# yeeus/GCI

Measured on AMD Instinct MI355X. Metric: aligned Gbases/s through filter+depth pipeline (CHM13, 40x HiFi), higher is better.
Workload: dtype int32

## Files before the change

### gci_amd/csrc/gci_wave.hpp

```cpp
#pragma once
#include <hip/hip_runtime.h>
#include <stdint.h>

template <int CTRL, int ROW_MASK>
__device__ __forceinline__ int32_t dpp_add(int32_t v)
{
    return v + __builtin_amdgcn_update_dpp(0, v, CTRL, ROW_MASK, 0xF, true);
}

__device__ __forceinline__ int32_t wave_inclusive_i32(int32_t v)
{
    v = dpp_add<0x111, 0xF>(v);
    v = dpp_add<0x112, 0xF>(v);
    v = dpp_add<0x114, 0xF>(v);
    v = dpp_add<0x118, 0xF>(v);
    v = dpp_add<0x142, 0xA>(v);
    v = dpp_add<0x143, 0xC>(v);
    return v;
}

template <typename T>
__device__ __forceinline__ T wave_inclusive(T v, int lane)
{
    if constexpr (sizeof(T) == 4) {
        return (T)wave_inclusive_i32((int32_t)v);
    } else {
#pragma unroll
        for (int d = 1; d < 64; d <<= 1) { T n = __shfl_up(v, d, 64); if (lane >= d) v += n; }
        return v;
    }
}

template <typename T>
__device__ __forceinline__ T wave_sum(T v)
{
    if constexpr (sizeof(T) == 4) {
        return (T)__builtin_amdgcn_readlane(wave_inclusive_i32((int32_t)v), 63);
    } else {
#pragma unroll
        for (int m = 32; m >= 1; m >>= 1) v += __shfl_xor(v, m, 64);
        return v;
    }
}

template <typename T, int NWAVES>
__device__ __forceinline__ T block_exclusive(T v, T* wtot, T& total)
{
    const int t = threadIdx.x, lane = t & 63, wave = t >> 6;
    const T inc = wave_inclusive<T>(v, lane);
    if (lane == 63) wtot[wave] = inc;
    __syncthreads();
    T pre = inc - v, all = 0;
#pragma unroll
    for (int w = 0; w < NWAVES; w++) { if (w < wave) pre += wtot[w]; all += wtot[w]; }
    total = all;
    return pre;
}
```

### gci_amd/csrc/k_filter.hip

```cpp
#include "gci_ctx.hpp"
#include <stdlib.h>

#ifndef G
#define G 4
#endif
#define NSLOT 10
#define LONG_OPS 512u
#ifndef HEAD
#define HEAD 112
#endif
#ifndef AUXB
#define AUXB 112
#endif
#define HEADP (HEAD + 16)
#define AUXP (AUXB + 16)
#define ROW (HEADP + AUXP)
#ifndef KB
#define KB 128
#endif
#ifndef NUP
#define NUP 8
#endif
#ifndef K1_WAVES
#define K1_WAVES 6
#endif
#if G == 4
#define GRP_STEPS(op) do { op(1); op(2); } while (0)
#else
#define GRP_STEPS(op) do { op(1); } while (0)
#endif

#define PIECES 8
#define CHUNK_DW (64 * PIECES * 4)

struct LongItem {
    uint64_t ops_off;
    uint32_t n_ops;
    uint32_t rec;
    int64_t nm;
    int32_t pos, contig, l_seq, n_cigar_field;
    uint32_t mapq;
    uint32_t n_chunks;
    uint32_t chunk_base;
    uint32_t pad;
};

struct ChunkSums { unsigned long long v[5]; };

struct LongQueue {
    uint32_t* next_counters;
    unsigned long long* status_in;
    unsigned long long* next_status;
    uint32_t* n_slow;
    unsigned long long* n_long;
    uint32_t* slow_list;
    LongItem* items;
    unsigned long long* chunks;
    ChunkSums* sums;
    uint32_t cap_items, cap_chunks;
    uint32_t has_seq;
};

__device__ __forceinline__ void report(unsigned long long* status, uint32_t rec, int code)
{
    atomicMin(status, ((unsigned long long)rec << 8) | (unsigned long long)(uint8_t)(-code));
}

__device__ __forceinline__ bool has_zero_byte(uint32_t x) { return ((x - 0x01010101u) & ~x & 0x80808080u) != 0; }

__device__ __forceinline__ bool ratio_cmp(int64_t a, int64_t b, double c, bool le)
{
    if (((a < 0 ? -a : a) | b) >> 30 == 0) {
        const float x = (float)(int32_t)a * __builtin_amdgcn_rcpf((float)(int32_t)b);
        const float cf = (float)c, m = 1e-4f * fmaxf(1.0f, fabsf(x));
        if (c == c && fabs(c) < 1e30) {
            if (x < cf - m) return le;
            if (x > cf + m) return !le;
        }
    }
    const double q = (double)a / (double)b;
    return le ? q <= c : q >= c;
}

__device__ __forceinline__ int decide4(gci_rec& r, int64_t S, int64_t den1, int64_t den2, int64_t rlen, bool have_nm,
                                       bool nm_bad_type, int64_t NM, int32_t pos, int32_t contig, int32_t l_seq,
                                       uint32_t n_cigar_field, int mapq, int mq_cutoff, double clip_percent,
                                       double iden_percent)
{
    if (!have_nm) return GCI_E_NO_NM;
    if (nm_bad_type) return GCI_E_BAD_NM_TYPE;
    if (den1 == 0) return GCI_E_ZERO_DIV;
    if (!ratio_cmp(S, den1, clip_percent, true)) return GCI_OK;
    if (den2 == 0) return GCI_E_ZERO_DIV;
    if (!ratio_cmp(den2 - NM, den2, iden_percent, false)) return GCI_OK;
    if (n_cigar_field == 0) return GCI_E_NO_END;
    r.contig = contig;
    r.start = pos;
    r.end = (int32_t)((int64_t)pos + (rlen > 0 ? rlen : 1));
    r.qlen = l_seq;
    r.flags = GCI_REC_PASS | (mapq >= mq_cutoff ? GCI_REC_HQ : 0);
    return GCI_OK;
}

__device__ __forceinline__ int decide(gci_rec& r, int64_t M, int64_t I, int64_t D, int64_t N, int64_t S, bool have_nm,
                                      bool nm_bad_type, int64_t NM, int32_t pos, int32_t contig, int32_t l_seq,
                                      uint32_t n_cigar_field, int mapq, int mq_cutoff, double clip_percent,
                                      double iden_percent)
{
    return decide4(r, S, M + I + S, M + I + D, M + D + N, have_nm, nm_bad_type, NM, pos, contig, l_seq, n_cigar_field, mapq, mq_cutoff,
                   clip_percent, iden_percent);
}

template <typename P>
__device__ __forceinline__ bool nm_value(P t, int64_t& NM)
{
    uint32_t w = 0;
    switch (t[0]) {
    case 'c': NM = (int8_t)t[1]; return true;
    case 'C': NM = t[1]; return true;
    case 's': w = (uint32_t)t[1] | ((uint32_t)t[2] << 8); NM = (int16_t)w; return true;
    case 'S': w = (uint32_t)t[1] | ((uint32_t)t[2] << 8); NM = w; return true;
    case 'i': w = (uint32_t)t[1] | ((uint32_t)t[2] << 8) | ((uint32_t)t[3] << 16) | ((uint32_t)t[4] << 24); NM = (int32_t)w; return true;
    case 'I': w = (uint32_t)t[1] | ((uint32_t)t[2] << 8) | ((uint32_t)t[3] << 16) | ((uint32_t)t[4] << 24); NM = w; return true;
    default: return false;
    }
}

__device__ __forceinline__ uint4 load16_tail(const uint8_t* __restrict__ bam, uint64_t at, uint64_t n_bytes)
{
    uint32_t w[4] = {0, 0, 0, 0};
#pragma unroll
    for (int i = 0; i < 16; i++) if (at + i < n_bytes) w[i >> 2] |= (uint32_t)bam[at + i] << (8 * (i & 3));
    return make_uint4(w[0], w[1], w[2], w[3]);
}

__device__ __forceinline__ void stage16(uint8_t* dst, const uint8_t* __restrict__ bam, uint64_t at, uint64_t n_bytes)
{
    uint4 v = make_uint4(0, 0, 0, 0);
    if (at + 16 <= n_bytes) v = *reinterpret_cast<const uint4*>(bam + at);
    else if (at < n_bytes) {
        v = load16_tail(bam, at, n_bytes);
    }
    *reinterpret_cast<uint4*>(dst) = v;
}

__device__ __forceinline__ uint32_t lds_u32(const uint8_t* p) { uint32_t v; __builtin_memcpy(&v, p, 4); return v; }

__device__ __forceinline__ void wave_lds_fence()
{
    __builtin_amdgcn_fence(__ATOMIC_RELEASE, "wavefront");
    __builtin_amdgcn_wave_barrier();
    __builtin_amdgcn_fence(__ATOMIC_ACQUIRE, "wavefront");
}

template <int W>
__device__ __forceinline__ bool enqueue_long(const LongQueue& q, LongItem it, int li)
{
    const uint32_t d0 = (uint32_t)(it.ops_off & 15ull) >> 2;
    const uint32_t nch = (uint32_t)(((uint64_t)d0 + it.n_ops + CHUNK_DW - 1) / CHUNK_DW);
    uint32_t slot, base;
    if (W == 64) {
        unsigned long long old = 0;
        if (li == 0) old = atomicAdd(q.n_long, (1ull << 32) | nch);
        slot = (uint32_t)__shfl((int)(old >> 32), 0, 64);
        base = (uint32_t)__shfl((int)(uint32_t)old, 0, 64);
    } else {
        const int lane = threadIdx.x & 63;
        const unsigned long long leaders = __ballot(li == 0);
        uint32_t items_below = 0, chunks_below = 0, chunks_all = 0;
        for (unsigned long long m = leaders; m; m &= m - 1ull) {
            const int l = __builtin_ctzll(m);
            const uint32_t v = (uint32_t)__shfl((int)nch, l, 64);
            if (l < (lane & ~(W - 1))) { items_below++; chunks_below += v; }
            chunks_all += v;
        }
        const int first = __builtin_ctzll(leaders);
        unsigned long long old = 0;
        if (lane == first) old = atomicAdd(q.n_long, ((unsigned long long)__builtin_popcountll(leaders) << 32) | chunks_all);
        slot = (uint32_t)__shfl((int)(old >> 32), first, 64) + items_below;
        base = (uint32_t)__shfl((int)(uint32_t)old, first, 64) + chunks_below;
    }
    const bool ok = slot < q.cap_items && (uint64_t)base + nch <= q.cap_chunks;
    if (li == 0 && slot < q.cap_items) {
        it.n_chunks = ok ? nch : 0u; it.chunk_base = base; it.pad = 0;
        q.items[slot] = it;
    }
    for (uint32_t c = li; c < nch; c += W)
        if ((uint64_t)base + c < q.cap_chunks) q.chunks[base + c] = ok ? ((unsigned long long)slot << 32) | c : ~0ull;
    return ok;
}


__device__ __forceinline__ void cigar_totals_wave(const uint8_t* __restrict__ bam, uint64_t n_bytes, uint64_t p0,
                                                  uint32_t n_ops, int lane, int64_t (&tot)[NSLOT])
{
    long long sum[NSLOT];
#pragma unroll
    for (int k = 0; k < NSLOT; k++) sum[k] = 0;
    const uint32_t sh = (uint32_t)(p0 & 15ull), d = sh >> 2, b = sh & 3u;
    const uint64_t a0 = p0 & ~15ull, lim = n_bytes & ~15ull;
    for (uint32_t c0 = lane; 4ull * c0 < n_ops; c0 += 256) {
        uint4 lo[4], hi[4];
#pragma unroll
        for (int u = 0; u < 4; u++) {
            const uint32_t c = c0 + 64u * u;
            const uint64_t a = a0 + 16ull * c;
            const bool in = 4ull * c < n_ops;
            lo[u] = !in ? make_uint4(0, 0, 0, 0) : a < lim ? *reinterpret_cast<const uint4*>(bam + a) : load16_tail(bam, a, n_bytes);
            hi[u] = !in ? make_uint4(0, 0, 0, 0) : a + 16 < lim ? *reinterpret_cast<const uint4*>(bam + a + 16) : load16_tail(bam, a + 16, n_bytes);
        }
#pragma unroll
        for (int u = 0; u < 4; u++) {
            const uint32_t c = c0 + 64u * u;
            if (4ull * c >= n_ops) continue;
            const uint32_t w[8] = {lo[u].x, lo[u].y, lo[u].z, lo[u].w, hi[u].x, hi[u].y, hi[u].z, hi[u].w};
            const uint32_t m = min(4u, n_ops - 4u * c);
#pragma unroll
            for (int j = 0; j < 4; j++) {
                const uint32_t x0 = d == 0 ? w[j] : d == 1 ? w[j + 1] : d == 2 ? w[j + 2] : w[j + 3];
                const uint32_t x1 = d == 0 ? w[j + 1] : d == 1 ? w[j + 2] : d == 2 ? w[j + 3] : w[j + 4];
                const uint32_t v = __builtin_amdgcn_alignbyte(x1, x0, b);
                const uint32_t op = v & 0xFu;
                const long long len = (uint32_t)j < m ? (long long)(v >> 4) : 0;
#pragma unroll
                for (int q = 0; q < NSLOT - 1; q++) sum[q] += op == (uint32_t)q ? len : 0;
            }
        }
    }
#pragma unroll
    for (int k = 0; k < NSLOT - 1; k++) tot[k] = wave_sum<long long>(sum[k]);
    tot[NSLOT - 1] = 0;
}


__device__ __forceinline__ uint32_t rd16b(const uint8_t* p) { return (uint32_t)p[0] | ((uint32_t)p[1] << 8); }
__device__ __forceinline__ uint32_t rd32b(const uint8_t* p) { return rd16b(p) | (rd16b(p + 2) << 16); }

__device__ __forceinline__ int64_t aux_value_size(const uint8_t* p, const uint8_t* end, uint8_t t)
{
    switch (t) {
    case 'A': case 'c': case 'C': return 1;
    case 's': case 'S': return 2;
    case 'i': case 'I': case 'f': return 4;
    case 'Z': case 'H': {
        const uint8_t* q = p;
        while (q < end && *q) q++;
        return q < end ? (q - p) + 1 : -1;
    }
    case 'B': {
        if (p + 5 > end) return -1;
        const uint8_t sub = p[0];
        const int64_t n = rd32b(p + 1);
        const int64_t es = (sub == 'c' || sub == 'C') ? 1 : (sub == 's' || sub == 'S') ? 2
                         : (sub == 'i' || sub == 'I' || sub == 'f') ? 4 : -1;
        return es < 0 ? -1 : 5 + n * es;
    }
    default: return -1;
    }
}

template <bool QUEUE_ALL = false>
__device__ __forceinline__ void slow_record(
    const uint8_t* __restrict__ bam, uint64_t n_bytes, const uint64_t off,
    const int32_t* __restrict__ ref_sel, uint32_t rec, int lane, const LongQueue& lq, int mq_cutoff, double clip_percent,
    double iden_percent, uint32_t rec_idx_base, gci_rec* __restrict__ out)
{
    const uint8_t* p = bam + off;
    const int32_t block_size = (int32_t)rd32b(p);
    const int32_t ref_id = (int32_t)rd32b(p + 4);
    const int32_t pos = (int32_t)rd32b(p + 8);
    const uint32_t l_read_name = p[12];
    const int mapq = p[13];
    const uint32_t n_cigar = rd16b(p + 16);
    const int32_t l_seq = (int32_t)rd32b(p + 20);
    const int32_t contig = ref_sel[ref_id];
    const uint8_t* name = p + 36;
    const uint8_t* rec_end = p + 4 + block_size;
    const uint8_t* cig = name + l_read_name;
    const uint8_t* aux = cig + 4 * (uint64_t)n_cigar + (lq.has_seq ? (((uint64_t)(uint32_t)l_seq + 1) >> 1) + (uint64_t)(uint32_t)l_seq : 0ull);
    uint32_t nul = l_read_name;
    for (uint32_t i = lane; i < l_read_name; i += 64) if (name[i] == 0) { nul = i; break; }
#pragma unroll
    for (int m = 32; m >= 1; m >>= 1) nul = min(nul, (uint32_t)__shfl_xor((int)nul, m, 64));
    const uint32_t name_len = nul;
    uint64_t acc = 0;
    for (uint32_t k = lane; k * 8 < name_len; k += 64) {
        uint64_t w = 0;
        for (int b = 0; b < 8; b++) if (k * 8 + b < name_len) w |= (uint64_t)name[k * 8 + b] << (8 * b);
        acc += gci_hash_word(w, k);
    }
    acc = (uint64_t)wave_sum<long long>((long long)acc);
    const uint8_t* nm_p = nullptr;
    const uint8_t* cg_p = nullptr;
    for (const uint8_t* q = aux; q + 3 <= rec_end;) {
        const int64_t sz = aux_value_size(q + 3, rec_end, q[2]);
        if (sz < 0 || q + 3 + sz > rec_end) break;
        if (q[0] == 'N' && q[1] == 'M' && !nm_p) nm_p = q + 2;
        if (q[0] == 'C' && q[1] == 'G' && !cg_p) cg_p = q + 2;
        q += 3 + sz;
// ... 247 lines not shown
    GRP_STEPS(STEP_ACC);
#undef STEP_ACC
    r.name_hash = gci_hash_finish(acc, name_len);
    r.name_len = (uint16_t)name_len;

    TR(6);
    if (long_cigar) {
        LongItem it;
        it.ops_off = off + cig_at; it.n_ops = n_cigar; it.rec = rec;
        it.nm = have_nm ? (nm_bad ? INT64_MIN : NM) : INT64_MAX;
        it.pos = pos; it.contig = contig; it.l_seq = l_seq; it.n_cigar_field = (int32_t)n_cigar;
        it.mapq = (uint32_t)mapq;
        if (gl == 0) out[rec] = r;
        if (!enqueue_long<G>(lq, it, gl) && gl == 0) report(lq.status_in, rec, GCI_E_CAPACITY);
        return false;
    }
#define GRP_SUM(x) do { x += (unsigned long long)__shfl_xor((long long)x, 1, G); if (G == 4) x += (unsigned long long)__shfl_xor((long long)x, 2, G); } while (0)
    GRP_SUM(sS); GRP_SUM(sQ); GRP_SUM(sA); GRP_SUM(sR);
#undef GRP_SUM
    if (gl != 0) return false;
    const int st = decide4(r, (int64_t)sS, (int64_t)sQ, (int64_t)sA, (int64_t)sR, have_nm, nm_bad, NM, pos, contig, l_seq,
                           n_cigar, mapq, mq_cutoff, clip_percent, iden_percent);
    if (st != GCI_OK) report(lq.status_in, rec, st);
    out[rec] = r;
    TR(7);
    return false;
    };
    const bool is_slow = live && fast_path();
    for (unsigned long long m = __ballot(is_slow && gl == 0); m; m &= m - 1ull) {
        const uint32_t rs = (uint32_t)__shfl((int)rec, __builtin_ctzll(m), 64);
        slow_record(bam, n_bytes, rec_off[rs], ref_sel, rs, t & 63, lq, mq_cutoff, clip_percent, iden_percent, rec_idx_base, out);
    }
}


__device__ __forceinline__ unsigned long long wave_sum_u40(unsigned long long v)
{
    const uint32_t lo = wave_sum<uint32_t>((uint32_t)v & 0xFFFFu);
    const uint32_t hi = wave_sum<uint32_t>((uint32_t)(v >> 16));
    return (unsigned long long)lo + ((unsigned long long)hi << 16);
}

__global__ __launch_bounds__(BLOCK) void k_cigar_chunks(const uint8_t* __restrict__ bam, uint64_t n_bytes, const LongQueue lq,
                                                        unsigned long long* __restrict__ status)
{
    if (blockIdx.x == 0 && threadIdx.x == 0) *status = *lq.status_in;
    const int lane = threadIdx.x & 63;
    const uint32_t n = (uint32_t)min((unsigned long long)(uint32_t)*lq.n_long, (unsigned long long)lq.cap_chunks);
    const uint32_t waves = gridDim.x * (BLOCK / 64);
    for (uint32_t wi = blockIdx.x * (BLOCK / 64) + (threadIdx.x >> 6); wi < n; wi += waves) {
        const unsigned long long e = lq.chunks[wi];
        if (e == ~0ull) continue;
        const LongItem* it = lq.items + (uint32_t)(e >> 32);
        const uint32_t ci = (uint32_t)e;
        const uint64_t p0 = it->ops_off;
        const uint32_t n_ops = it->n_ops;
        const uint32_t d0 = (uint32_t)(p0 & 15ull) >> 2, b = (uint32_t)p0 & 3u;
        const uint64_t g0 = (uint64_t)ci * CHUNK_DW;
        const uint64_t abase = (p0 & ~15ull) + g0 * 4ull;
        const uint32_t r0 = ci == 0 ? d0 : 0u;
        const uint32_t r1 = (uint32_t)min((uint64_t)CHUNK_DW, (uint64_t)d0 + n_ops - g0);
        uint4 pc[PIECES];
#pragma unroll
        for (int u = 0; u < PIECES; u++) {
            const uint32_t c = lane + 64u * u;
            const uint64_t at = abase + 16ull * c;
            const bool need = 4u * c < r1 + 1u && 4u * c + 4u > r0;
            pc[u] = !need ? make_uint4(0, 0, 0, 0) : at + 16 <= n_bytes ? *reinterpret_cast<const uint4*>(bam + at)
                                                                          : load16_tail(bam, at, n_bytes);
        }
        uint32_t ext = 0;
        if (r1 == CHUNK_DW && b != 0) {
            const uint64_t at = abase + 4ull * CHUNK_DW;
            ext = at + 4 <= n_bytes ? *reinterpret_cast<const uint32_t*>(bam + at) : load16_tail(bam, at, n_bytes).x;
        }
        unsigned long long wide[5] = {0ull, 0ull, 0ull, 0ull, 0ull};
        uint32_t s[5] = {0u, 0u, 0u, 0u, 0u};
#pragma unroll
        for (int u = 0; u < PIECES; u++) {
            uint32_t w4 = (uint32_t)__shfl((int)pc[u].x, (lane + 1) & 63, 64);
            const uint32_t first_next = u + 1 < PIECES ? (uint32_t)__builtin_amdgcn_readfirstlane((int)pc[(u + 1) % PIECES].x) : ext;
            if (lane == 63) w4 = first_next;
            const uint32_t w[5] = {pc[u].x, pc[u].y, pc[u].z, pc[u].w, w4};
            const uint32_t li0 = 4u * (lane + 64u * u);
#pragma unroll
            for (int j = 0; j < 4; j++) {
                const uint32_t v = __builtin_amdgcn_alignbyte(w[j + 1], w[j], b);
                const uint32_t len = (li0 + j - r0) < (r1 - r0) ? v >> 4 : 0u;
                const uint32_t op = v & 0xFu;
                s[0] += len & (0u - ((0x181u >> op) & 1u));
                s[1] += op == 1u ? len : 0u;
                s[2] += op == 2u ? len : 0u;
                s[3] += op == 3u ? len : 0u;
                s[4] += op == 4u ? len : 0u;
            }
            if ((u & 3) == 3) {
#pragma unroll
                for (int k = 0; k < 5; k++) { wide[k] += s[k]; s[k] = 0u; }
            }
        }
        ChunkSums out;
#pragma unroll
        for (int k = 0; k < 5; k++) out.v[k] = wave_sum_u40(wide[k]);
        if (lane == 0) lq.sums[wi] = out;
    }
}

__global__ __launch_bounds__(BLOCK) void k_cigar_finish(const LongQueue lq, int mq_cutoff, double clip_percent,
                                                        double iden_percent, gci_rec* __restrict__ out,
                                                        unsigned long long* __restrict__ status)
{
    const uint32_t n = (uint32_t)min(*lq.n_long >> 32, (unsigned long long)lq.cap_items);
    for (uint32_t i = blockIdx.x * BLOCK + threadIdx.x; i < n; i += gridDim.x * BLOCK) {
        const LongItem x = lq.items[i];
        if (x.n_chunks == 0) continue;
        int64_t t[5] = {0, 0, 0, 0, 0};
        for (uint32_t c = 0; c < x.n_chunks; c++) {
            const ChunkSums cs = lq.sums[x.chunk_base + c];
#pragma unroll
            for (int k = 0; k < 5; k++) t[k] += (int64_t)cs.v[k];
        }
        gci_rec r = out[x.rec];
        const int st = decide(r, t[0], t[1], t[2], t[3], t[4], x.nm != INT64_MAX, x.nm == INT64_MIN, x.nm, x.pos, x.contig,
                              x.l_seq, (uint32_t)x.n_cigar_field, (int)(x.mapq & 0xFFu), mq_cutoff, clip_percent, iden_percent);
        if (st != GCI_OK) report(status, x.rec, st);
        if (r.flags) r.flags |= (uint8_t)(x.mapq >> 8);
        out[x.rec] = r;
    }
}

#define PGK 256
#define PG_KIND_EXT 1u
#define PG_KIND_OVERSIZE 2u
#define PG_KIND_MALFORMED 4u
#define PG_MAGIC 0x31504347u
#define PG_REF_LDS 1024

struct PagesArgs {
    const uint8_t* buf; uint64_t total_bytes; uint32_t page_bytes, n_pages, n_rec;
    const int32_t* ref_sel; int32_t n_ref; int map_qual, mq_cutoff; double clip_percent, iden_percent;
    uint32_t rec_idx_base; gci_rec* out; uint64_t* name_off;
};

#ifndef PG_LPR
#define PG_LPR 4
#endif
#ifndef PG_WAVES
#define PG_WAVES 5
#endif
__global__ __launch_bounds__(PGK) __attribute__((amdgpu_waves_per_eu(PG_WAVES, PG_WAVES))) void k_bam_filter_pages(const PagesArgs A, const LongQueue lq)
{
    extern __shared__ __attribute__((aligned(16))) uint8_t page[];
    __shared__ uint8_t aux_sz[256];
    __shared__ uint8_t aux_kind[256];
    __shared__ uint16_t s_full[GCI_PAGE_MAX_BYTES / 48];
    __shared__ uint32_t s_n_full;
    __shared__ int32_t s_ref_sel[PG_REF_LDS];
    const int t = threadIdx.x;
    const bool ref_in_lds = A.n_ref <= PG_REF_LDS;
    if (ref_in_lds) for (int i = t; i < A.n_ref; i += PGK) s_ref_sel[i] = A.ref_sel[i];
    if (t == 0) s_n_full = 0;
    if (blockIdx.x == 0 && t < 4) lq.next_counters[t] = 0u;
    if (blockIdx.x == 0 && t == 4) *lq.next_status = ~0ull;
    const uint32_t P = A.page_bytes;
    const uint64_t page_at = (uint64_t)blockIdx.x * P;
    {
        const uint4* __restrict__ src = reinterpret_cast<const uint4*>(A.buf + page_at);
        const uint32_t rounds = P / (16u * PGK);
        for (uint32_t r0 = 0; r0 < rounds; r0 += 8) {
            uint4 v[8];
#pragma unroll
            for (int u = 0; u < 8; u++) v[u] = r0 + u < rounds ? src[(r0 + u) * PGK + t] : make_uint4(0, 0, 0, 0);
#pragma unroll
            for (int u = 0; u < 8; u++) if (r0 + u < rounds) reinterpret_cast<uint4*>(page)[(r0 + u) * PGK + t] = v[u];
        }
    }
    for (int i = t; i < 256; i += PGK) {
        const char c = (char)i;
        aux_sz[i] = (c == 'A' || c == 'c' || c == 'C') ? 1 : (c == 's' || c == 'S') ? 2 : (c == 'i' || c == 'I' || c == 'f') ? 4 : 0;
        aux_kind[i] = aux_sz[i] | ((c == 'c' || c == 's' || c == 'i') ? 8 : 0) | ((c == 'c' || c == 'C' || c == 's' || c == 'S' || c == 'i' || c == 'I') ? 16 : 0);
    }
    __syncthreads();
    const uint32_t* ph = reinterpret_cast<const uint32_t*>(page);
    uint32_t n_recs = ph[0];
    const uint32_t first_rec = ph[1];
    if (ph[3] != PG_MAGIC || n_recs > (P - 16u) / 50u || (uint64_t)first_rec + n_recs > A.n_rec) {
        if (t == 0) report(lq.status_in, first_rec < A.n_rec ? first_rec : 0u, GCI_E_MALFORMED);
        n_recs = 0;
    }
    {
        const int tv = PG_LPR == 4 ? t : (int)(((uint32_t)t + 64u * (blockIdx.x & 3u)) & (PGK - 1u));
        const int gl = tv % PG_LPR;
        const uint32_t lgrp = (uint32_t)tv / PG_LPR;
        for (uint32_t j0 = 0; j0 < n_recs; j0 += PGK / PG_LPR) {
            const uint32_t j = j0 + lgrp;
            const uint32_t rec = first_rec + j;
            auto lean_path = [&]() -> int {
                uint32_t base = (uint32_t)reinterpret_cast<const uint16_t*>(page + 16)[j] << 4;
                if (base > P - 48u) return 1;
                const uint8_t* hd = page + base;
                const uint4 c0 = *reinterpret_cast<const uint4*>(hd);
                const uint4 c1 = *reinterpret_cast<const uint4*>(hd + 16);
                const uint32_t size = c0.x, kind = c0.w >> 16, l_read_name = c0.w & 0xFFu, n_cigar = c1.x & 0xFFFFu, flag = c1.x >> 16;
                const int32_t ref_id = (int32_t)c0.y, pos = (int32_t)c0.z, l_seq = (int32_t)c1.y;
                const int mapq = (int)((c0.w >> 8) & 0xFFu);
                const uint32_t aux_len = c1.z;
                const uint32_t cig_at = (36u + l_read_name + 15u) & ~15u;
                const uint32_t aux_at = cig_at + ((4u * n_cigar + 15u) & ~15u);
                if (kind != 0 || l_read_name == 0 || n_cigar == 0 || (uint64_t)aux_at + aux_len > size || base + size > P) return 1;
                gci_rec r;
                r.name_hash = 0; r.contig = -1; r.start = 0; r.end = 0; r.qlen = 0; r.rec_idx = rec + A.rec_idx_base;
                r.mapq = (uint8_t)mapq; r.flags = 0; r.name_len = 0;
                if (gl == 0 && A.name_off) A.name_off[rec] = page_at + base + 36u;
                int32_t contig = -1;
                if (!(ref_id < 0 || ref_id >= A.n_ref || (flag & (0x4u | 0x100u | 0x800u)) || mapq < A.map_qual))
                    contig = ref_in_lds ? s_ref_sel[ref_id] : A.ref_sel[ref_id];
                if (contig < 0) {
                    if (gl == 0) A.out[rec] = r;
                    return 0;
                }
                const uint32_t op0 = lds_u32(hd + cig_at);
                if (pos >= 0 && (op0 & 0xFu) == 4u && (op0 >> 4) == (uint32_t)l_seq) return 1;
                uint32_t sS = 0, sQ = 0, sA = 0, sR = 0, big = 0;
                auto add_op = [&](uint32_t v) {
                    const uint32_t op = v & 0xFu, len = v >> 4;
                    sS = __umul24(len, __builtin_amdgcn_ubfe(0x010u, op, 1)) + sS;
                    sQ = __umul24(len, __builtin_amdgcn_ubfe(0x193u, op, 1)) + sQ;
                    sA = __umul24(len, __builtin_amdgcn_ubfe(0x187u, op, 1)) + sA;
                    sR = __umul24(len, __builtin_amdgcn_ubfe(0x18Du, op, 1)) + sR;
                };
                {
                    const uint8_t* cg = hd + cig_at;
                    for (uint32_t p = gl; 4u * p < n_cigar; p += PG_LPR) {
                        const uint4 v = *reinterpret_cast<const uint4*>(cg + 16u * p);
                        big |= v.x | v.y | v.z | v.w;
                        add_op(v.x); add_op(v.y); add_op(v.z); add_op(v.w);
                    }
                }
                const uint8_t* ax = hd + aux_at;
                uint32_t q = 0, nmk = 0;
                for (;;) {
                    if (q + 3 > aux_len) return 1;
                    const uint32_t w = lds_u32(ax + q);
                    const uint32_t k = aux_kind[(w >> 16) & 0xFFu];
                    if ((k & 7u) == 0 || q + 3 + (k & 7u) > aux_len) return 1;
                    if ((w & 0xFFFFu) == (uint32_t)('N' | ('M' << 8))) { nmk = k; break; }
                    q += 3 + (k & 7u);
                }
                if (!(nmk & 16u)) return 1;
                const uint32_t nv = lds_u32(ax + q + 3), nbits = 8u * (nmk & 7u);
                const int64_t NM = nbits == 32u ? ((nmk & 8u) ? (int64_t)(int32_t)nv : (int64_t)nv)
                                                : ((nmk & 8u) ? (int64_t)__builtin_amdgcn_sbfe((int)nv, 0, nbits) : (int64_t)__builtin_amdgcn_ubfe(nv, 0, nbits));
                const uint8_t* name = hd + 36;
                const uint32_t name_len = l_read_name - 1u;
                bool odd = name[name_len] != 0;
                uint64_t acc = 0;
                for (uint32_t k = gl; k * 8 < name_len; k += PG_LPR) {
                    const uint32_t b0 = k * 8;
                    uint64_t w;
                    __builtin_memcpy(&w, name + b0, 8);
                    const uint32_t keep = name_len - b0;
                    if (keep < 8) w &= (1ull << (8 * keep)) - 1ull;
                    const uint64_t full = keep < 8 ? w | (~0ull << (8 * keep)) : w;
                    odd = odd || (((full - 0x0101010101010101ull) & ~full & 0x8080808080808080ull) != 0);
                    acc += gci_hash_word(w, k);
                }
#pragma unroll
                for (int m = 1; m < PG_LPR; m <<= 1) acc += (uint64_t)__shfl_xor((long long)acc, m, PG_LPR);
                big |= odd ? 0xF0000000u : 0u;
#pragma unroll
                for (int m = 1; m < PG_LPR; m <<= 1) big |= (uint32_t)__shfl_xor((int)big, m, PG_LPR);
                if (big >> 28) return 1;
#define PG_SUM32(x) do { _Pragma("unroll") for (int m = 1; m < PG_LPR; m <<= 1) x += (uint32_t)__shfl_xor((int)x, m, PG_LPR); } while (0)
                PG_SUM32(sS); PG_SUM32(sQ); PG_SUM32(sA); PG_SUM32(sR);
#undef PG_SUM32
                const int64_t num2 = (int64_t)sA - NM;
                if (sQ == 0 || sA == 0 || (sQ >> 30) || (sA >> 30) || num2 > (1 << 30) || num2 < -(1 << 30)) return 1;
                const float x1 = (float)sS * __builtin_amdgcn_rcpf((float)sQ), c1f = (float)A.clip_percent;
                const float x2 = (float)(int32_t)num2 * __builtin_amdgcn_rcpf((float)sA), c2f = (float)A.iden_percent;
                const float m1 = 1e-4f * fmaxf(1.0f, fabsf(x1)), m2 = 1e-4f * fmaxf(1.0f, fabsf(x2));
                if (!(fabs(A.clip_percent) < 1e30) || !(fabs(A.iden_percent) < 1e30)) return 1;
                if (!(x1 < c1f - m1 || x1 > c1f + m1)) return 1;
                r.name_hash = gci_hash_finish(acc, name_len);
                r.name_len = (uint16_t)name_len;
                if (x1 < c1f - m1) {
                    if (!(x2 < c2f - m2 || x2 > c2f + m2)) return 1;
                    if (x2 > c2f + m2) {
                        r.contig = contig; r.start = pos;
                        r.end = (int32_t)((int64_t)pos + (sR > 0 ? (int64_t)sR : 1));
                        r.qlen = l_seq;
                        r.flags = GCI_REC_PASS | (mapq >= A.mq_cutoff ? GCI_REC_HQ : 0) | GCI_REC_NAME16;
                    }
                }
                if (gl == 0) A.out[rec] = r;
                return 0;
            };

            if (j < n_recs && lean_path() != 0 && gl == 0) s_full[atomicAdd(&s_n_full, 1u)] = (uint16_t)j;
        }
    }
    __syncthreads();
    const uint32_t n_full = s_n_full;
    const int gl = t & 3, grp = t >> 2;
    for (uint32_t q0 = 0; q0 < n_full; q0 += PGK / 4) {
        const uint32_t qi = q0 + grp;
        const bool on = qi < n_full;
        const uint32_t j = on ? s_full[qi] : 0u;
        const uint32_t rec = first_rec + j;
        uint64_t slow_off = 0;
        auto fast_path = [&]() -> bool {
            uint32_t base = (uint32_t)reinterpret_cast<const uint16_t*>(page + 16)[j] << 4;
            if (base > P - 48u) base = P - 48u;
            const uint8_t* hd = page + base;
            const uint4 c0 = *reinterpret_cast<const uint4*>(hd);
            const uint4 c1 = *reinterpret_cast<const uint4*>(hd + 16);
            const uint32_t blob_hi = *reinterpret_cast<const uint32_t*>(hd + 32);
            const uint32_t size = c0.x, kind = c0.w >> 16, l_read_name = c0.w & 0xFFu, n_cigar = c1.x & 0xFFFFu, flag = c1.x >> 16;
            const int32_t ref_id = (int32_t)c0.y, pos = (int32_t)c0.z, l_seq = (int32_t)c1.y;
            const int mapq = (int)((c0.w >> 8) & 0xFFu);
            const uint32_t aux_len = c1.z;
            const uint64_t blob_at = (uint64_t)c1.w | ((uint64_t)blob_hi << 32);
            gci_rec r;
            r.name_hash = 0; r.contig = -1; r.start = 0; r.end = 0; r.qlen = 0; r.rec_idx = rec + A.rec_idx_base;
            r.mapq = (uint8_t)mapq; r.flags = 0; r.name_len = 0;
            if (gl == 0 && A.name_off) A.name_off[rec] = (kind == PG_KIND_OVERSIZE ? blob_at : page_at + base) + 36u;
            const bool ext = kind == PG_KIND_EXT;
            const uint32_t cig_at = (36u + l_read_name + 15u) & ~15u;
            const uint32_t aux_at = cig_at + (ext ? 16u : (4u * n_cigar + 15u) & ~15u);
            if ((kind & PG_KIND_MALFORMED) || (kind != PG_KIND_OVERSIZE && ((uint64_t)aux_at + aux_len > size || base + size > P))) {
                if (gl == 0) { report(lq.status_in, rec, GCI_E_MALFORMED); A.out[rec] = r; }
                return false;
            }
            if (ref_id < 0 || ref_id >= A.n_ref || (flag & (0x4u | 0x100u | 0x800u)) || mapq < A.map_qual) {
                if (gl == 0) A.out[rec] = r;
                return false;
            }
            const int32_t contig = ref_in_lds ? s_ref_sel[ref_id] : A.ref_sel[ref_id];
            if (contig < 0) {
                if (gl == 0) A.out[rec] = r;
                return false;
            }
            if (kind == PG_KIND_OVERSIZE) {
                if (blob_at + 36 > A.total_bytes) { if (gl == 0) { report(lq.status_in, rec, GCI_E_MALFORMED); A.out[rec] = r; } return false; }
                slow_off = blob_at;
                return true;
            }
            uint32_t sS = 0, sQ = 0, sA = 0, sR = 0, big = 0;
            auto add_op = [&](uint32_t v) {
                const uint32_t op = v & 0xFu, len = v >> 4;
                sS = __umul24(len, __builtin_amdgcn_ubfe(0x010u, op, 1)) + sS;
                sQ = __umul24(len, __builtin_amdgcn_ubfe(0x193u, op, 1)) + sQ;
                sA = __umul24(len, __builtin_amdgcn_ubfe(0x187u, op, 1)) + sA;
                sR = __umul24(len, __builtin_amdgcn_ubfe(0x18Du, op, 1)) + sR;
            };
            if (!ext) {
                const uint8_t* cg = hd + cig_at;
                for (uint32_t p = gl; 4u * p < n_cigar; p += 4) {
                    const uint4 v = *reinterpret_cast<const uint4*>(cg + 16u * p);
                    big |= v.x | v.y | v.z | v.w;
                    add_op(v.x); add_op(v.y); add_op(v.z); add_op(v.w);
                }
            }
            const uint8_t* ax = hd + aux_at;
            const uint32_t op0 = lds_u32(hd + cig_at);
            const bool want_cg = n_cigar > 0 && pos >= 0 && (op0 & 0xFu) == 4u && (op0 >> 4) == (uint32_t)l_seq;
            bool have_nm = false, nm_bad = false;
            int64_t NM = 0;
            uint32_t cg_q = 0xFFFFFFFFu;
            uint32_t q = 0;
            bool general = want_cg;
            while (!general && q + 3 <= aux_len) {
                const uint32_t w = lds_u32(ax + q);
                const uint32_t sz = aux_sz[(w >> 16) & 0xFFu];
                if (sz == 0) { general = true; break; }
                if (q + 3 + sz > aux_len) break;
                if ((w & 0xFFFFu) == (uint32_t)('N' | ('M' << 8))) { have_nm = true; nm_bad = !nm_value(ax + q + 2, NM); break; }
                q += 3 + sz;
            }
            for (; general && q + 3 <= aux_len;) {
                const uint32_t w = lds_u32(ax + q);
                const uint32_t tag = w & 0xFFFFu;
                const uint8_t ty = (uint8_t)(w >> 16);
                uint32_t sz = aux_sz[ty];
                if (sz == 0) {
                    if (ty == 'Z' || ty == 'H') {
                        uint32_t e = q + 3;
                        while (e < aux_len && ax[e]) e++;
                        if (e >= aux_len) break;
                        sz = e - (q + 3) + 1;
                    } else if (ty == 'B') {
                        if (q + 8 > aux_len) break;
                        const uint8_t sub = ax[q + 3];
                        const uint32_t es = (sub == 'c' || sub == 'C') ? 1u : (sub == 's' || sub == 'S') ? 2u
                                          : (sub == 'i' || sub == 'I' || sub == 'f') ? 4u : 0u;
                        const uint64_t s64 = 5ull + (uint64_t)lds_u32(ax + q + 4) * es;
                        if (es == 0 || s64 > aux_len) break;
                        sz = (uint32_t)s64;
                    } else break;
                }
                if (q + 3 + sz > aux_len) break;
                if (tag == (uint32_t)('N' | ('M' << 8)) && !have_nm) {
                    have_nm = true;
                    nm_bad = !nm_value(ax + q + 2, NM);
                    if (!want_cg || cg_q != 0xFFFFFFFFu) break;
                }
                if (want_cg && tag == (uint32_t)('C' | ('G' << 8)) && cg_q == 0xFFFFFFFFu) {
                    cg_q = q + 2;
                    if (have_nm) break;
                }
                q += 3 + sz;
            }
            bool restored = false;
            if (cg_q != 0xFFFFFFFFu && ax[cg_q] == 'B' && (ax[cg_q + 1] == 'I' || ax[cg_q + 1] == 'i')) {
                const uint32_t cg_len = lds_u32(ax + cg_q + 2);
                if (cg_len >= n_cigar && cg_len < (1u << 29)) {
                    restored = true;
                    sS = sQ = sA = sR = 0; big = 0;
                    for (uint32_t k = gl; k < cg_len; k += 4) { const uint32_t v = lds_u32(ax + cg_q + 6 + 4 * k); big |= v; add_op(v); }
                }
            }
            const uint8_t* name = hd + 36;
            uint32_t nul = l_read_name;
            for (uint32_t i = gl * 4; i < l_read_name; i += 16) {
                if (has_zero_byte(lds_u32(name + i))) {
                    for (uint32_t b = i; b < i + 4 && b < l_read_name; b++) if (name[b] == 0) { nul = min(nul, b); break; }
                    break;
                }
            }
            nul = min(nul, (uint32_t)__shfl_xor((int)nul, 1, 4));
            nul = min(nul, (uint32_t)__shfl_xor((int)nul, 2, 4));
            const uint32_t name_len = nul;
            uint64_t acc = 0;
            for (uint32_t k = gl; k * 8 < name_len; k += 4) {
                const uint32_t b0 = k * 8;
                uint64_t w;
                __builtin_memcpy(&w, name + b0, 8);
                const uint32_t keep = name_len - b0;
                if (keep < 8) w &= (1ull << (8 * keep)) - 1ull;
                acc += gci_hash_word(w, k);
            }
            acc += (uint64_t)__shfl_xor((long long)acc, 1, 4);
            acc += (uint64_t)__shfl_xor((long long)acc, 2, 4);
            r.name_hash = gci_hash_finish(acc, name_len);
            r.name_len = (uint16_t)name_len;
            const uint8_t name16 = name_len + 1u == l_read_name ? GCI_REC_NAME16 : 0;
            big |= (uint32_t)__shfl_xor((int)big, 1, 4);
            big |= (uint32_t)__shfl_xor((int)big, 2, 4);
            const bool wide = (big >> 28) != 0 && !restored;
            if ((ext && !restored) || wide) {
                LongItem it;
                it.ops_off = ext ? blob_at : page_at + base + cig_at; it.n_ops = n_cigar; it.rec = rec;
                it.nm = have_nm ? (nm_bad ? INT64_MIN : NM) : INT64_MAX;
                it.pos = pos; it.contig = contig; it.l_seq = l_seq; it.n_cigar_field = (int32_t)n_cigar;
                it.mapq = (uint32_t)mapq | ((uint32_t)name16 << 8);
                r.flags = 0;
                if (gl == 0) A.out[rec] = r;
                if (it.ops_off + 4ull * n_cigar > A.total_bytes) { if (gl == 0) report(lq.status_in, rec, GCI_E_MALFORMED); return false; }
                if (!enqueue_long<4>(lq, it, gl) && gl == 0) report(lq.status_in, rec, GCI_E_CAPACITY);
                return false;
            }
            unsigned long long tS = sS, tQ = sQ, tA = sA, tR = sR;
            if ((big >> 28) != 0) {
                tS = tQ = tA = tR = 0;
                const uint32_t cg_len = lds_u32(ax + cg_q + 2);
                for (uint32_t k = gl; k < cg_len; k += 4) {
                    const uint32_t v = lds_u32(ax + cg_q + 6 + 4 * k), op = v & 0xFu;
                    const unsigned long long len = v >> 4;
                    tS += len & (0ull - ((0x010u >> op) & 1u)); tQ += len & (0ull - ((0x193u >> op) & 1u));
                    tA += len & (0ull - ((0x187u >> op) & 1u)); tR += len & (0ull - ((0x18Du >> op) & 1u));
                }
            }
#define PG_SUM(x) do { x += (unsigned long long)__shfl_xor((long long)x, 1, 4); x += (unsigned long long)__shfl_xor((long long)x, 2, 4); } while (0)
            PG_SUM(tS); PG_SUM(tQ); PG_SUM(tA); PG_SUM(tR);
#undef PG_SUM
            if (gl != 0) return false;
            const int st = decide4(r, (int64_t)tS, (int64_t)tQ, (int64_t)tA, (int64_t)tR, have_nm, nm_bad, NM, pos, contig, l_seq,
                                   n_cigar, mapq, A.mq_cutoff, A.clip_percent, A.iden_percent);
            if (st != GCI_OK) report(lq.status_in, rec, st);
            if (r.flags) r.flags |= name16;
            A.out[rec] = r;
            return false;
        };
        const bool is_slow = on && fast_path();
        for (unsigned long long m = __ballot(is_slow && gl == 0); m; m &= m - 1ull) {
            const int l = __builtin_ctzll(m);
            const uint32_t rs = (uint32_t)__shfl((int)rec, l, 64);
            const uint64_t so = (uint64_t)__shfl((long long)slow_off, l, 64);
            slow_record<true>(A.buf, A.total_bytes, so, A.ref_sel, rs, t & 63, lq, A.mq_cutoff, A.clip_percent, A.iden_percent, A.rec_idx_base, A.out);
        }
    }
// ... 116 lines not shown
```

Baseline: 24260.

## Restructure lean BAM filter path with batched LDS loads and quad DPP reductions

Rewrites the per-record lean filter path so all LDS loads (contig lookup, first CIGAR op, first CIGAR vector, aux word, NM value, name terminator, first name word) are issued up front and held in registers with clamped addresses. CIGAR and name loops are software-pipelined with prefetch of the next element. Group reductions use quad DPP swizzles instead of shfl_xor, the aux type lookup table is replaced by bitmask arithmetic, and the pass is specialised on whether ref_sel fits in LDS. Records are written as two 16-byte halves by two lanes when the output is aligned. The intent is to cut LDS latency serialisation and branch divergence, at the cost of more registers and speculative loads.

Measured after the change: 24250. About the same (-0.0%).

```diff
diff --git a/gci_amd/csrc/gci_wave.hpp b/gci_amd/csrc/gci_wave.hpp
--- a/gci_amd/csrc/gci_wave.hpp
+++ b/gci_amd/csrc/gci_wave.hpp
@@ -43,6 +43,30 @@
     }
 }
 
+template <int CTRL>
+__device__ __forceinline__ uint32_t quad_get(uint32_t v)
+{
+    return (uint32_t)__builtin_amdgcn_update_dpp(0, (int32_t)v, CTRL, 0xF, 0xF, true);
+}
+
+__device__ __forceinline__ uint32_t quad_sum(uint32_t v)
+{
+    v += quad_get<0xB1>(v);
+    return v + quad_get<0x4E>(v);
+}
+
+__device__ __forceinline__ uint32_t quad_or(uint32_t v)
+{
+    v |= quad_get<0xB1>(v);
+    return v | quad_get<0x4E>(v);
+}
+
+__device__ __forceinline__ uint64_t quad_sum(uint64_t v)
+{
+    v += (uint64_t)quad_get<0xB1>((uint32_t)v) | ((uint64_t)quad_get<0xB1>((uint32_t)(v >> 32)) << 32);
+    return v + ((uint64_t)quad_get<0x4E>((uint32_t)v) | ((uint64_t)quad_get<0x4E>((uint32_t)(v >> 32)) << 32));
+}
+
 template <typename T, int NWAVES>
 __device__ __forceinline__ T block_exclusive(T v, T* wtot, T& total)
 {
diff --git a/gci_amd/csrc/k_filter.hip b/gci_amd/csrc/k_filter.hip
--- a/gci_amd/csrc/k_filter.hip
+++ b/gci_amd/csrc/k_filter.hip
@@ -145,6 +145,7 @@
 }
 
 __device__ __forceinline__ uint32_t lds_u32(const uint8_t* p) { uint32_t v; __builtin_memcpy(&v, p, 4); return v; }
+__device__ __forceinline__ int32_t lds_i32(const int32_t* p) { return *(const __attribute__((address_space(3))) int32_t*)p; }
 
 __device__ __forceinline__ void wave_lds_fence()
 {
@@ -698,7 +699,6 @@
 {
     extern __shared__ __attribute__((aligned(16))) uint8_t page[];
     __shared__ uint8_t aux_sz[256];
-    __shared__ uint8_t aux_kind[256];
     __shared__ uint16_t s_full[GCI_PAGE_MAX_BYTES / 48];
     __shared__ uint32_t s_n_full;
     __shared__ int32_t s_ref_sel[PG_REF_LDS];
@@ -724,8 +724,10 @@
     for (int i = t; i < 256; i += PGK) {
         const char c = (char)i;
         aux_sz[i] = (c == 'A' || c == 'c' || c == 'C') ? 1 : (c == 's' || c == 'S') ? 2 : (c == 'i' || c == 'I' || c == 'f') ? 4 : 0;
-        aux_kind[i] = aux_sz[i] | ((c == 'c' || c == 's' || c == 'i') ? 8 : 0) | ((c == 'c' || c == 'C' || c == 's' || c == 'S' || c == 'i' || c == 'I') ? 16 : 0);
-    }
+    }
+    const bool thr_ok = fabs(A.clip_percent) < 1e30 && fabs(A.iden_percent) < 1e30;
+    const float c1f = (float)A.clip_percent, c2f = (float)A.iden_percent;
+    const bool out16 = (reinterpret_cast<uintptr_t>(A.out) & 15u) == 0;
     __syncthreads();
     const uint32_t* ph = reinterpret_cast<const uint32_t*>(page);
     uint32_t n_recs = ph[0];
@@ -738,112 +740,153 @@
         const int tv = PG_LPR == 4 ? t : (int)(((uint32_t)t + 64u * (blockIdx.x & 3u)) & (PGK - 1u));
         const int gl = tv % PG_LPR;
         const uint32_t lgrp = (uint32_t)tv / PG_LPR;
-        for (uint32_t j0 = 0; j0 < n_recs; j0 += PGK / PG_LPR) {
-            const uint32_t j = j0 + lgrp;
-            const uint32_t rec = first_rec + j;
-            auto lean_path = [&]() -> int {
-                uint32_t base = (uint32_t)reinterpret_cast<const uint16_t*>(page + 16)[j] << 4;
-                if (base > P - 48u) return 1;
-                const uint8_t* hd = page + base;
-                const uint4 c0 = *reinterpret_cast<const uint4*>(hd);
-                const uint4 c1 = *reinterpret_cast<const uint4*>(hd + 16);
-                const uint32_t size = c0.x, kind = c0.w >> 16, l_read_name = c0.w & 0xFFu, n_cigar = c1.x & 0xFFFFu, flag = c1.x >> 16;
-                const int32_t ref_id = (int32_t)c0.y, pos = (int32_t)c0.z, l_seq = (int32_t)c1.y;
-                const int mapq = (int)((c0.w >> 8) & 0xFFu);
-                const uint32_t aux_len = c1.z;
-                const uint32_t cig_at = (36u + l_read_name + 15u) & ~15u;
-                const uint32_t aux_at = cig_at + ((4u * n_cigar + 15u) & ~15u);
-                if (kind != 0 || l_read_name == 0 || n_cigar == 0 || (uint64_t)aux_at + aux_len > size || base + size > P) return 1;
-                gci_rec r;
-                r.name_hash = 0; r.contig = -1; r.start = 0; r.end = 0; r.qlen = 0; r.rec_idx = rec + A.rec_idx_base;
-                r.mapq = (uint8_t)mapq; r.flags = 0; r.name_len = 0;
-                if (gl == 0 && A.name_off) A.name_off[rec] = page_at + base + 36u;
-                int32_t contig = -1;
-                if (!(ref_id < 0 || ref_id >= A.n_ref || (flag & (0x4u | 0x100u | 0x800u)) || mapq < A.map_qual))
-                    contig = ref_in_lds ? s_ref_sel[ref_id] : A.ref_sel[ref_id];
-                if (contig < 0) {
-                    if (gl == 0) A.out[rec] = r;
-                    return 0;
-                }
-                const uint32_t op0 = lds_u32(hd + cig_at);
-                if (pos >= 0 && (op0 & 0xFu) == 4u && (op0 >> 4) == (uint32_t)l_seq) return 1;
-                uint32_t sS = 0, sQ = 0, sA = 0, sR = 0, big = 0;
-                auto add_op = [&](uint32_t v) {
-                    const uint32_t op = v & 0xFu, len = v >> 4;
-                    sS = __umul24(len, __builtin_amdgcn_ubfe(0x010u, op, 1)) + sS;
-                    sQ = __umul24(len, __builtin_amdgcn_ubfe(0x193u, op, 1)) + sQ;
-                    sA = __umul24(len, __builtin_amdgcn_ubfe(0x187u, op, 1)) + sA;
-                    sR = __umul24(len, __builtin_amdgcn_ubfe(0x18Du, op, 1)) + sR;
-                };
-                {
-                    const uint8_t* cg = hd + cig_at;
+        auto grp_sum = [](uint32_t x) -> uint32_t {
+            if constexpr (PG_LPR == 4) return quad_sum(x);
+#pragma unroll
+            for (int m = 1; m < PG_LPR; m <<= 1) x += (uint32_t)__shfl_xor((int)x, m, PG_LPR);
+            return x;
+        };
+        auto grp_or = [](uint32_t x) -> uint32_t {
+            if constexpr (PG_LPR == 4) return quad_or(x);
+#pragma unroll
+            for (int m = 1; m < PG_LPR; m <<= 1) x |= (uint32_t)__shfl_xor((int)x, m, PG_LPR);
+            return x;
+        };
+        auto grp_sum64 = [](uint64_t x) -> uint64_t {
+            if constexpr (PG_LPR == 4) return quad_sum(x);
+#pragma unroll
+            for (int m = 1; m < PG_LPR; m <<= 1) x += (uint64_t)__shfl_xor((long long)x, m, PG_LPR);
+            return x;
+        };
+        auto put_rec = [&](const gci_rec& r, uint32_t rec, uint32_t base) {
+            constexpr int NL = PG_LPR >= 4 ? 2 : 0;
+            if (out16 && PG_LPR >= 2) {
+                const bool up = gl != 0;
+                const uint32_t tail = (uint32_t)r.mapq | ((uint32_t)r.flags << 8) | ((uint32_t)r.name_len << 16);
+                const uint4 half = make_uint4(up ? (uint32_t)r.end : (uint32_t)r.name_hash, up ? (uint32_t)r.qlen : (uint32_t)(r.name_hash >> 32),
+                                              up ? r.rec_idx : (uint32_t)r.contig, up ? tail : (uint32_t)r.start);
+                if (gl < 2) reinterpret_cast<uint4*>(A.out)[2 * (size_t)rec + gl] = half;
+            } else if (gl == 0) A.out[rec] = r;
+            if (gl == NL && A.name_off) A.name_off[rec] = page_at + base + 36u;
+        };
+        auto lean_pass = [&](auto in_lds) {
+            for (uint32_t j0 = 0; j0 < n_recs; j0 += PGK / PG_LPR) {
+                const uint32_t j = j0 + lgrp;
+                const uint32_t rec = first_rec + j;
+                auto lean_path = [&]() -> int {
+                    const uint32_t base0 = (uint32_t)reinterpret_cast<const uint16_t*>(page + 16)[j] << 4;
+                    const uint32_t base = min(base0, P - 48u);
+                    const uint8_t* hd = page + base;
+                    const uint4 c0 = *reinterpret_cast<const uint4*>(hd);
+                    const uint4 c1 = *reinterpret_cast<const uint4*>(hd + 16);
+                    uint64_t nw;
+                    __builtin_memcpy(&nw, page + min(base + 36u + 8u * (uint32_t)gl, P - 8u), 8);
+                    const uint32_t size = c0.x, kind = c0.w >> 16, l_read_name = c0.w & 0xFFu, flag = c1.x >> 16;
+                    const int32_t ref_id = (int32_t)c0.y, pos = (int32_t)c0.z, l_seq = (int32_t)c1.y;
+                    const int mapq = (int)((c0.w >> 8) & 0xFFu);
+                    const uint32_t n_cigar = c1.x & 0xFFFFu, aux_len = c1.z;
+                    const uint32_t cig_at = (36u + l_read_name + 15u) & ~15u;
+                    const uint32_t aux_at = cig_at + ((4u * n_cigar + 15u) & ~15u);
+                    if (base0 > P - 48u || kind != 0 || l_read_name == 0 || n_cigar == 0 || (uint64_t)aux_at + aux_len > size || size > P - base)
+                        return 1;
+                    const uint32_t name_len = l_read_name - 1u;
+                    const bool filtered = ref_id < 0 || ref_id >= A.n_ref || (flag & (0x4u | 0x100u | 0x800u)) || mapq < A.map_qual;
+                    const uint32_t cg_at = base + cig_at, ax_at = base + aux_at;
+                    int32_t contig = -1;
+                    if constexpr (decltype(in_lds)::value) contig = lds_i32(s_ref_sel + (filtered ? 0 : ref_id));
+                    else if (!filtered) contig = A.ref_sel[ref_id];
+                    uint32_t op0 = lds_u32(page + min(cg_at, P - 4u));
+                    uint4 cv = *reinterpret_cast<const uint4*>(page + min(cg_at + 16u * (uint32_t)gl, P - 16u));
+                    uint32_t w = lds_u32(page + min(ax_at, P - 4u));
+                    uint32_t nv_at = min(ax_at + 3u, P - 4u);
+                    uint32_t nv = lds_u32(page + nv_at);
+                    uint32_t nul = page[min(base + 36u + name_len, P - 1u)];
+                    asm volatile("" : "+v"(contig), "+v"(op0), "+v"(w), "+v"(nv), "+v"(nul), "+v"(cv.x), "+v"(cv.y), "+v"(cv.z), "+v"(cv.w));
+                    bool odd = nul != 0;
+                    if (filtered) contig = -1;
+                    gci_rec r;
+                    r.name_hash = 0; r.contig = -1; r.start = 0; r.end = 0; r.qlen = 0; r.rec_idx = rec + A.rec_idx_base;
+                    r.mapq = (uint8_t)mapq; r.flags = 0; r.name_len = 0;
+                    if (contig < 0) {
+                        put_rec(r, rec, base);
+                        return 0;
+                    }
+                    bool leave = pos >= 0 && (op0 & 0xFu) == 4u && (op0 >> 4) == (uint32_t)l_seq;
+                    uint32_t sS = 0, sQ = 0, sA = 0, sR = 0, big = 0;
+                    auto add_op = [&](uint32_t v) {
+                        const uint32_t op = v & 0xFu, len = v >> 4;
+                        sS = __umul24(len, __builtin_amdgcn_ubfe(0x010u, op, 1)) + sS;
+                        sQ = __umul24(len, __builtin_amdgcn_ubfe(0x193u, op, 1)) + sQ;
+                        sA = __umul24(len, __builtin_amdgcn_ubfe(0x187u, op, 1)) + sA;
+                        sR = __umul24(len, __builtin_amdgcn_ubfe(0x18Du, op, 1)) + sR;
+                    };
                     for (uint32_t p = gl; 4u * p < n_cigar; p += PG_LPR) {
-                        const uint4 v = *reinterpret_cast<const uint4*>(cg + 16u * p);
-                        big |= v.x | v.y | v.z | v.w;
-                        add_op(v.x); add_op(v.y); add_op(v.z); add_op(v.w);
+                        const uint4 nx = *reinterpret_cast<const uint4*>(page + min(cg_at + 16u * (p + PG_LPR), P - 16u));
+                        big |= cv.x | cv.y | cv.z | cv.w;
+                        add_op(cv.x); add_op(cv.y); add_op(cv.z); add_op(cv.w);
+                        cv = nx;
                     }
-                }
-                const uint8_t* ax = hd + aux_at;
-                uint32_t q = 0, nmk = 0;
-                for (;;) {
-                    if (q + 3 > aux_len) return 1;
-                    const uint32_t w = lds_u32(ax + q);
-                    const uint32_t k = aux_kind[(w >> 16) & 0xFFu];
-                    if ((k & 7u) == 0 || q + 3 + (k & 7u) > aux_len) return 1;
-                    if ((w & 0xFFFFu) == (uint32_t)('N' | ('M' << 8))) { nmk = k; break; }
-                    q += 3 + (k & 7u);
-                }
-                if (!(nmk & 16u)) return 1;
-                const uint32_t nv = lds_u32(ax + q + 3), nbits = 8u * (nmk & 7u);
-                const int64_t NM = nbits == 32u ? ((nmk & 8u) ? (int64_t)(int32_t)nv : (int64_t)nv)
-                                                : ((nmk & 8u) ? (int64_t)__builtin_amdgcn_sbfe((int)nv, 0, nbits) : (int64_t)__builtin_amdgcn_ubfe(nv, 0, nbits));
-                const uint8_t* name = hd + 36;
-                const uint32_t name_len = l_read_name - 1u;
-                bool odd = name[name_len] != 0;
-                uint64_t acc = 0;
-                for (uint32_t k = gl; k * 8 < name_len; k += PG_LPR) {
-                    const uint32_t b0 = k * 8;
-                    uint64_t w;
-                    __builtin_memcpy(&w, name + b0, 8);
-                    const uint32_t keep = name_len - b0;
-                    if (keep < 8) w &= (1ull << (8 * keep)) - 1ull;
-                    const uint64_t full = keep < 8 ? w | (~0ull << (8 * keep)) : w;
-                    odd = odd || (((full - 0x0101010101010101ull) & ~full & 0x8080808080808080ull) != 0);
-                    acc += gci_hash_word(w, k);
-                }
-#pragma unroll
-                for (int m = 1; m < PG_LPR; m <<= 1) acc += (uint64_t)__shfl_xor((long long)acc, m, PG_LPR);
-                big |= odd ? 0xF0000000u : 0u;
-#pragma unroll
-                for (int m = 1; m < PG_LPR; m <<= 1) big |= (uint32_t)__shfl_xor((int)big, m, PG_LPR);
-                if (big >> 28) return 1;
-#define PG_SUM32(x) do { _Pragma("unroll") for (int m = 1; m < PG_LPR; m <<= 1) x += (uint32_t)__shfl_xor((int)x, m, PG_LPR); } while (0)
-                PG_SUM32(sS); PG_SUM32(sQ); PG_SUM32(sA); PG_SUM32(sR);
-#undef PG_SUM32
-                const int64_t num2 = (int64_t)sA - NM;
-                if (sQ == 0 || sA == 0 || (sQ >> 30) || (sA >> 30) || num2 > (1 << 30) || num2 < -(1 << 30)) return 1;
-                const float x1 = (float)sS * __builtin_amdgcn_rcpf((float)sQ), c1f = (float)A.clip_percent;
-                const float x2 = (float)(int32_t)num2 * __builtin_amdgcn_rcpf((float)sA), c2f = (float)A.iden_percent;
-                const float m1 = 1e-4f * fmaxf(1.0f, fabsf(x1)), m2 = 1e-4f * fmaxf(1.0f, fabsf(x2));
-                if (!(fabs(A.clip_percent) < 1e30) || !(fabs(A.iden_percent) < 1e30)) return 1;
-                if (!(x1 < c1f - m1 || x1 > c1f + m1)) return 1;
-                r.name_hash = gci_hash_finish(acc, name_len);
-                r.name_len = (uint16_t)name_len;
-                if (x1 < c1f - m1) {
-                    if (!(x2 < c2f - m2 || x2 > c2f + m2)) return 1;
-                    if (x2 > c2f + m2) {
+                    uint32_t q = 0, nmk = 0;
+                    leave = leave || aux_len < 3u;
+                    for (bool on = !leave; on;) {
+                        const uint32_t ty = (w >> 16) & 0xFFu, lo5 = ty & 31u, blk = ty >> 5;
+                        const uint32_t known = blk == 2u ? 0x8020Au : blk == 3u ? 0x80248u : 0u;
+                        const uint32_t sz = __builtin_amdgcn_ubfe(0xAu, lo5, 1) | (__builtin_amdgcn_ubfe(0x80000u, lo5, 1) << 1) |
+                                            (__builtin_amdgcn_ubfe(0x240u, lo5, 1) << 2);
+                        const uint32_t in = __builtin_amdgcn_ubfe(0x80208u, lo5, 1);
+                        if (!__builtin_amdgcn_ubfe(known, lo5, 1) || q + 3 + sz > aux_len) { leave = true; break; }
+                        if ((w & 0xFFFFu) == (uint32_t)('N' | ('M' << 8))) { nmk = sz | ((in & blk) << 3) | (in << 4); break; }
+                        q += 3 + sz;
+                        if (q + 3 > aux_len) { leave = true; break; }
+                        w = lds_u32(page + ax_at + q);
+                        nv_at = min(ax_at + q + 3u, P - 4u);
+                        nv = lds_u32(page + nv_at);
+                    }
+                    leave = leave || !(nmk & 16u);
+                    nv >>= (8u * (ax_at + q + 3u - nv_at)) & 31u;
+                    const uint32_t nbits = 8u * (nmk & 7u);
+                    const int64_t NM = nbits == 32u ? ((nmk & 8u) ? (int64_t)(int32_t)nv : (int64_t)nv)
+                                                    : ((nmk & 8u) ? (int64_t)__builtin_amdgcn_sbfe((int)nv, 0, nbits) : (int64_t)__builtin_amdgcn_ubfe(nv, 0, nbits));
+                    uint64_t acc = 0;
+                    for (uint32_t k = gl; k * 8 < name_len; k += PG_LPR) {
+                        uint64_t nx;
+                        __builtin_memcpy(&nx, page + min(base + 36u + 8u * (k + PG_LPR), P - 8u), 8);
+                        const uint32_t keep = name_len - k * 8;
+                        uint64_t wd = nw;
+                        if (keep < 8) wd &= (1ull << (8 * keep)) - 1ull;
+                        const uint64_t full = keep < 8 ? wd | (~0ull << (8 * keep)) : wd;
+                        odd = odd || (((full - 0x0101010101010101ull) & ~full & 0x8080808080808080ull) != 0);
+                        acc += gci_hash_word(wd, k);
+                        nw = nx;
+                    }
+                    acc = grp_sum64(acc);
+                    big |= odd ? 0xF0000000u : 0u;
+                    big = grp_or(big);
+                    sS = grp_sum(sS); sQ = grp_sum(sQ); sA = grp_sum(sA); sR = grp_sum(sR);
+                    const int64_t num2 = (int64_t)sA - NM;
+                    leave = leave || (big >> 28) || !thr_ok || sQ == 0 || sA == 0 || (sQ >> 30) || (sA >> 30) || num2 > (1 << 30) || num2 < -(1 << 30);
+                    const float x1 = (float)sS * __builtin_amdgcn_rcpf((float)sQ);
+                    const float x2 = (float)(int32_t)num2 * __builtin_amdgcn_rcpf((float)sA);
+                    const float m1 = 1e-4f * fmaxf(1.0f, fabsf(x1)), m2 = 1e-4f * fmaxf(1.0f, fabsf(x2));
+                    const bool clip_ok = x1 < c1f - m1, iden_ok = x2 > c2f + m2;
+                    leave = leave || !(clip_ok || x1 > c1f + m1) || (clip_ok && !(iden_ok || x2 < c2f - m2));
+                    if (leave) return 1;
+                    r.name_hash = gci_hash_finish(acc, name_len);
+                    r.name_len = (uint16_t)name_len;
+                    if (clip_ok && iden_ok) {
                         r.contig = contig; r.start = pos;
                         r.end = (int32_t)((int64_t)pos + (sR > 0 ? (int64_t)sR : 1));
                         r.qlen = l_seq;
                         r.flags = GCI_REC_PASS | (mapq >= A.mq_cutoff ? GCI_REC_HQ : 0) | GCI_REC_NAME16;
                     }
-                }
-                if (gl == 0) A.out[rec] = r;
-                return 0;
-            };
-
-            if (j < n_recs && lean_path() != 0 && gl == 0) s_full[atomicAdd(&s_n_full, 1u)] = (uint16_t)j;
-        }
+                    put_rec(r, rec, base);
+                    return 0;
+                };
+
+                if (j < n_recs && lean_path() != 0 && gl == 0) s_full[atomicAdd(&s_n_full, 1u)] = (uint16_t)j;
+            }
+        };
+        if (ref_in_lds) lean_pass(std::true_type()); else lean_pass(std::false_type());
     }
     __syncthreads();
     const uint32_t n_full = s_n_full;
@@ -881,7 +924,8 @@
                 if (gl == 0) A.out[rec] = r;
                 return false;
             }
-            const int32_t contig = ref_in_lds ? s_ref_sel[ref_id] : A.ref_sel[ref_id];
+            int32_t contig;
+            if (ref_in_lds) contig = lds_i32(s_ref_sel + ref_id); else contig = A.ref_sel[ref_id];
             if (contig < 0) {
                 if (gl == 0) A.out[rec] = r;
                 return false;
```
